# zacharie12/Hypernet-image-captioning

Hardware: AMD Instinct MI355X
Metric: training images/sec at 1/2/4/8 MI355X, Flickr30k GRU+hypernet bs=128 (higher is better)
Workload: dtype f32; 1 GPU; Flickr30k-shaped GRU+additive-attention decoder + hypernet (3 style domains), full training step (fwd, CE, bwd, clip 5.0, Adam); per_gpu_batch=128, global_batch=128, T=20, P=49, D=2048, F=200, E=200, H=200, V=9684, hypernet_params=144906720, parallelism=dp1, launch=eager, next_theta_in_adam_pass=True, next_precompute_beside_adam=True, spinup_steps=0, deterministic_gradients=True

## Files before the change

hypernet-image-captioning_amd/csrc/decoder.hip:

```cpp
#include "common.h"
#include "decoder_internal.h"
#include "gemm_internal.h"
#include <algorithm>
#include <initializer_list>
#include <mutex>

int g_tune_deterministic = 0;
int g_tune_rec_pair = 1;
int g_tune_rec_rotate = 1;
int g_tune_vocab_order = 1;
int g_tune_branch_mask = 7;
int g_tune_splitk_target = 1280;
int g_tune_chain_main = 0;
int g_tune_hops = 0;
int g_tune_fork = 4;
int g_tune_join_chain = 0;
int g_tune_sk_dhs = 0, g_tune_sk_vocab_w = 0;
#define RUN(x) do { int _rc = (x); if (_rc != CAPHN_OK) return _rc; } while (0)

namespace {

struct Side {
    hipStream_t st[3];
    enum { D_FORK = 0, D_JOIN = 1, D_X = 4, D_MS = 10, D_PRE_F = 14, D_PRE_ALL = 15, D_COUNT = 16 };
    struct Dep { hipEvent_t ev; unsigned seq = 0; bool by_value = false; };
    Dep deps[D_COUNT];
    unsigned* vals = nullptr;
    unsigned counter = 0;
    bool values = false;
    bool pre_valid = false;
    const void* pre_ws = nullptr;
    bool ready = false, on = false;
    bool forked[3] = {false, false, false};
    hipStream_t main = nullptr;
    int init() {
        if (ready) return CAPHN_OK;
        static std::mutex mu;
        std::lock_guard<std::mutex> lock(mu);
        if (ready) return CAPHN_OK;
        for (auto& s : st) if (hipStreamCreateWithFlags(&s, hipStreamNonBlocking) != hipSuccess) return CAPHN_ELAUNCH;
        for (auto& d : deps) if (hipEventCreateWithFlags(&d.ev, hipEventDisableTiming) != hipSuccess) return CAPHN_ELAUNCH;
        void* p = nullptr;
        if (hipMalloc(&p, sizeof(unsigned) * D_COUNT) == hipSuccess && hipMemset(p, 0, sizeof(unsigned) * D_COUNT) == hipSuccess)
            vals = static_cast<unsigned*>(p);
        else (void)hipGetLastError();
        ready = true;
        return CAPHN_OK;
    }
    int post(int slot, hipStream_t from) {
// ... 54 lines not shown
        return await(D_JOIN + i, st[j]);
    }
    struct Scope {
        Side& s;
        explicit Scope(Side& side) : s(side) {}
        ~Scope() { for (int i = 0; i < 3; ++i) if (s.on && s.forked[i]) (void)s.jointo(i); }
    };
    hipStream_t xfrom[6] = {nullptr, nullptr, nullptr, nullptr, nullptr, nullptr};
    int record(int k, hipStream_t from) {
        if (!on) return CAPHN_OK;
        xfrom[k] = from;
        return post(D_X + k, from);
    }
    int wait(int k, hipStream_t to) {
        if (!on || xfrom[k] == to) return CAPHN_OK;
        return await(D_X + k, to);
    }
    int dep(hipStream_t from, hipStream_t to, int k) {
        if (!on || from == to) return CAPHN_OK;
        if (post(D_X + k, from) != CAPHN_OK) return CAPHN_ELAUNCH;
        return await(D_X + k, to);
    }
};
constexpr int MAX_DEVICES = 64;
Side g_sides[MAX_DEVICES];
inline Side* side_here() {
    int dev = 0;
    if (hipGetDevice(&dev) != hipSuccess || dev < 0 || dev >= MAX_DEVICES) return nullptr;
    return &g_sides[dev];
}

struct Ws {
    size_t Y1, f, meanf, h0, c0, Waf, G, Xe, Xg, Hs, Hprev, gates, hn, Cs, Cprev, uah, alphas, idx;
    size_t dHs, dgi, dgh, duah, de, dh0, dc0, ctx, dctx, dXe, dWaf, dmeanf, df, dY1, apart, vtmp, colws, colws_s[3], prof, rowmap;
    size_t xch, xch_floats;
    size_t wp;
    size_t H0s, dH0, h0L, dcarry, tgi, tgh, tmpA, tmpB;
    size_t Lin[CAPHN_MAX_DEC_LAYERS - 1], Lgates[CAPHN_MAX_DEC_LAYERS - 1], Lhn[CAPHN_MAX_DEC_LAYERS - 1],
           Ldgi[CAPHN_MAX_DEC_LAYERS - 1], Ldgh[CAPHN_MAX_DEC_LAYERS - 1];
    int L1;
    size_t total;
    int npc, pchunk, NG, arows;
};
inline bool use_pair(const caphn_decoder_dims* d) {
    const int NG = d->cell == CAPHN_CELL_LSTM ? 4 : 3;
    return g_tune_rec_pair && d->T > 1 && d->layers <= 1 && caphn_rec_pair_resident_gates(d->P, d->H, NG) >= 0;
}

inline size_t up4(size_t v) { return (v + 3) & ~(size_t)3; }

inline Ws layout(const caphn_decoder_dims* d) {
    Ws w;
    const size_t B = d->B, T = d->T, P = d->P, F = d->F, E = d->E, H = d->H, V = d->V, D = d->D;
    const bool lstm = d->cell == CAPHN_CELL_LSTM, raw = d->raw_features != 0;
    const size_t NG = lstm ? 4 : 3;
    w.NG = (int)NG;
    size_t o = 0;
    auto take = [&](size_t n) { size_t r = o; o += up4(n); return r; };
    w.Y1 = take(raw ? 0 : B * P * F); w.f = take(raw ? 0 : B * P * F); w.meanf = take(B * F); w.h0 = take(B * H);
    w.c0 = take(lstm ? B * H : 0);
    w.Waf = take(B * P * H); w.G = take(B * P * NG * H); w.Xe = take(B * T * (E + F)); w.Xg = take(B * T * NG * H);
    w.Hs = take(B * T * H); w.Hprev = take(B * T * H); w.gates = take(B * T * NG * H); w.hn = take(lstm ? 0 : B * T * H);
    w.Cs = take(lstm ? B * T * H : 0); w.Cprev = take(lstm ? B * T * H : 0);
    w.uah = take(B * T * H); w.alphas = take(B * T * P); w.idx = take(2 * B * T);
    w.dHs = take(B * T * H); w.dgi = take(B * T * NG * H); w.dgh = take(lstm ? 0 : B * T * NG * H); w.duah = take(B * T * H);
    w.de = take(B * T * P); w.dh0 = take(B * H); w.dc0 = take(lstm ? B * H : 0);
    w.ctx = w.Xe + E; w.dctx = take(raw ? 0 : B * T * F);
    w.dXe = take(B * T * E); w.dWaf = take(B * P * H); w.dmeanf = take(raw ? 0 : 2 * B * F); w.df = take(raw ? 0 : B * P * F);
    w.dY1 = take(raw ? 0 : B * P * F);
    w.pchunk = 1; w.npc = (int)((P + w.pchunk - 1) / w.pchunk);
    const size_t arows = std::max<size_t>(std::max<size_t>(w.npc, (size_t)caphn_rec_bwd_groups((int)P, (int)H)),
                                          (size_t)caphn_rec_pair_bwd_groups((int)P, (int)H));
    w.arows = (int)arows;
    w.apart = take(B * arows * (H + 1)); w.vtmp = take(H + 1);
    size_t cs = 0;
    auto need = [&](size_t M, size_t N) { cs = std::max(cs, caphn_colsum_workspace_bytes((int)M, (int)N) / sizeof(float)); };
    need(B * T, V); need(B * T, NG * H); need(B * T, H); need(B * P, H); need(B * P, F); need(B, H);
    need(B * arows, H + 1);
    if (d->layers > 1) need(B * (T + 1), 3 * H);
    w.colws = take(cs);
    {
        size_t c2 = 0;
        auto need2 = [&](size_t M, size_t N) { c2 = std::max(c2, caphn_colsum_workspace_bytes((int)M, (int)N) / sizeof(float)); };
        need2(B * T, NG * H); need2(B * T, H); need2(B * P, H); need2(B * P, F); need2(B, H); need2(B * arows, H + 1);
        if (d->layers > 1) need2(B * (T + 1), 3 * H);
        for (int i = 0; i < 3; ++i) w.colws_s[i] = take(c2);
    }
    w.prof = take(64);
    w.rowmap = take(B * T + 4);
    w.xch_floats = caphn_rec_pair_xch_bytes((int)B, (int)P, (int)H) / sizeof(float);
    w.xch = take(2 * w.xch_floats);
    o = (o + 31) & ~(size_t)31;
    w.wp = take(caphn_rec_pair_wp_floats((int)H, (int)NG));
    w.L1 = d->layers > 1 ? d->layers - 1 : 0;
    {
        const size_t on = w.L1 > 0 ? 1 : 0, S = T + 1;
        w.H0s = take(on * B * T * H); w.dH0 = take(on * B * T * H); w.h0L = take(on * B * H); w.dcarry = take(on * B * H);
        w.tgi = take(on * B * 3 * H); w.tgh = take(on * B * 3 * H); w.tmpA = take(on * B * H); w.tmpB = take(on * B * H);
        for (int l = 0; l < CAPHN_MAX_DEC_LAYERS - 1; ++l) {
            const size_t u = l < w.L1 ? 1 : 0;
            w.Lin[l] = take(u * B * S * H); w.Lgates[l] = take(u * B * S * 3 * H); w.Lhn[l] = take(u * B * S * H);
            w.Ldgi[l] = take(u * B * S * 3 * H); w.Ldgh[l] = take(u * B * S * 3 * H);
        }
    }
    w.total = o;
    (void)D;
    return w;
}

__global__ __launch_bounds__(1024) void valid_rows_kernel(int n, const int64_t* __restrict__ tgt, int64_t ignore, int* __restrict__ map) {
    __shared__ int wsum[16];
    __shared__ int base_s;
    const int tid = threadIdx.x, lane = tid & 63, wave = tid >> 6;
    if (tid == 0) base_s = 0;
    __syncthreads();
    for (int c0 = 0; c0 < n; c0 += 1024) {
        const int i = c0 + tid;
        const int v = (i < n && tgt[i] != ignore) ? 1 : 0;
        const unsigned long long ball = __ballot(v);
        const int before = __popcll(ball & ((1ull << lane) - 1ull));
        if (lane == 0) wsum[wave] = __popcll(ball);
        __syncthreads();
        int woff = 0, tot = 0;
        for (int q = 0; q < 16; ++q) { if (q < wave) woff += wsum[q]; tot += wsum[q]; }
        const int base = base_s;
        if (v) map[4 + base + woff + before] = i;
        __syncthreads();
        if (tid == 0) base_s = base + tot;
        __syncthreads();
    }
    if (tid == 0) map[0] = base_s;
}

__global__ void copy2_kernel(const float* __restrict__ src, int n, float* __restrict__ a, float* __restrict__ b) {
    const int i = blockIdx.x * blockDim.x + threadIdx.x;
    if (i < n) a[i] = src[i];
    else if (i == n) b[0] = src[n];
}

__global__ __launch_bounds__(256) void teacher_inputs_kernel(int T, int E, const int64_t* __restrict__ caps, const float* __restrict__ table,
                                                            int64_t* __restrict__ idx, float* __restrict__ out, int ostride) {
    const int i = blockIdx.x, t = i % T;
    const int64_t id = t < 2 ? (int64_t)-1 : caps[i - 1];
    if (threadIdx.x == 0) idx[i] = id;
    for (int e = threadIdx.x; e < E; e += 256) out[(size_t)i * ostride + e] = id < 0 ? 0.f : table[(size_t)id * E + e];
}

inline bool dims_ok(const caphn_decoder_dims* d) {
    if (d && !(d->dropout_p >= 0.f && d->dropout_p < 1.f)) return false;
    if (!(d && d->B > 0 && d->T > 0 && d->P > 0 && d->D > 0 && d->F > 0 && d->E > 0 && d->H > 0 && d->V > 0)) return false;
    if (d->cell != CAPHN_CELL_GRU && d->cell != CAPHN_CELL_LSTM) return false;
    if (d->raw_features && d->F != d->D) return false;
    if (d->layers < 0 || d->layers > CAPHN_MAX_DEC_LAYERS) return false;
    if (d->layers > 1 && d->cell != CAPHN_CELL_GRU) return false;
    if (d->logits_ld != 0 && d->logits_ld < d->V) return false;
    return true;
}
inline bool layer_params_ok(const caphn_decoder_dims* d, const caphn_decoder_params* p) {
    for (int l = 0; l + 1 < d->layers; ++l)
        if (!p->lw_ih[l] || !p->lw_hh[l] || !p->lb_ih[l] || !p->lb_hh[l]) return false;
    return true;
}

inline int pick_splitk(int M, int N, int K) {
// ... 129 lines not shown
        a.dgi = ws + w.Ldgi[l]; a.dgh = ws + w.Ldgh[l]; a.dout = o; a.dout_ld = o_ld;
        if (l == w.L1 - 1 && slot > 0) { a.drop_p = d->dropout_p; a.drop_seed = d->dropout_seed; a.T = d->T; a.t = slot - 1; }
        RUN(caphn_launch_layer_gru_bwd(a, s));
        RUN(caphn_gemm_f32(0, 0, B, H, G3, ws + w.Ldgi[l] + (size_t)slot * G3, S * G3, p->lw_ih[l], H, o, o_ld, nullptr, nullptr, 0,
                           CAPHN_GEMM_ACCUM, 1, s));
        RUN(caphn_gemm_f32(0, 0, B, H, G3, ws + w.Ldgh[l] + (size_t)slot * G3, S * G3, p->lw_hh[l], H, o, o_ld, nullptr, nullptr, 0,
                           CAPHN_GEMM_ACCUM, 1, s));
        d1 = o; d1_ld = o_ld; d2 = nullptr;
    }
    return CAPHN_OK;
}

}

extern "C" size_t caphn_decoder_workspace_bytes(const caphn_decoder_dims* d) {
    if (!dims_ok(d)) return 0;
    return layout(d).total * sizeof(float);
}

extern "C" const int* caphn_decoder_rowcount_ptr(const caphn_decoder_dims* d, void* ws_) {
    if (!dims_ok(d) || !ws_) return nullptr;
    return reinterpret_cast<const int*>(static_cast<float*>(ws_) + layout(d).rowmap);
}

extern "C" unsigned long long* caphn_decoder_profile_ptr(const caphn_decoder_dims* d, void* ws_) {
    if (!dims_ok(d) || !ws_) return nullptr;
    return reinterpret_cast<unsigned long long*>(static_cast<float*>(ws_) + layout(d).prof);
}

extern "C" int caphn_decoder_prepare_rows(const caphn_decoder_dims* d, const int64_t* targets, int64_t ignore_index,
                                          void* ws_, caphn_stream_t stream) {
    if (!dims_ok(d) || !targets || !ws_) return CAPHN_EINVAL;
    const Ws w = layout(d);
    hipLaunchKernelGGL(valid_rows_kernel, dim3(1), dim3(1024), 0, static_cast<hipStream_t>(stream), d->B * d->T, targets,
                       ignore_index, reinterpret_cast<int*>(static_cast<float*>(ws_) + w.rowmap));
    return caphn_launch_status();
}

static int decoder_inputs(const caphn_decoder_dims* d, const caphn_decoder_params* p, const Ws& w, float* ws,
                          const int64_t* captions, hipStream_t s, int parts = 3) {
    const int BT = d->B * d->T, E = d->E, GH = w.NG * d->H, EF = d->E + d->F;
    int64_t* idx = reinterpret_cast<int64_t*>(ws + w.idx);
    if ((parts & 1) && !(d->precomputed & 64))
        hipLaunchKernelGGL(teacher_inputs_kernel, dim3(BT), dim3(256), 0, s, d->T, E, captions, p->embed_w, idx, ws + w.Xe, EF);
    if (parts & 2)
    RUN(caphn_gemm_f32(0, 1, BT, GH, E, ws + w.Xe, EF, p->w_ih, EF, ws + w.Xg, GH, p->b_ih, nullptr, 0, CAPHN_GEMM_BIAS, 1, s));
    return CAPHN_OK;
}

extern "C" int caphn_decoder_precompute(const caphn_decoder_dims* d, const caphn_decoder_params* p, const float* features,
                                        const int64_t* captions, void* ws_, caphn_stream_t stream) {
    if (!dims_ok(d) || !p || !features || !ws_) return CAPHN_EINVAL;
    const bool raw = d->raw_features != 0;
    if (!raw && (!p->fc0_w || !p->fc0_b || !p->fc2_w || !p->fc2_b)) return CAPHN_EINVAL;
    if (d->cell == CAPHN_CELL_LSTM && (!p->initc_w || !p->initc_b)) return CAPHN_EINVAL;
    const Ws w = layout(d);
    hipStream_t s = static_cast<hipStream_t>(stream);
    const float* f = nullptr;
    RUN(decoder_precompute(d, p, w, static_cast<float*>(ws_), features, &f, s, (captions ? 3 : 1) & ~(d->precomputed & 1), true));
    if (captions && !(d->precomputed & 4)) RUN(decoder_inputs(d, p, w, static_cast<float*>(ws_), captions, s));
    Side* sd = side_here();
    if (!sd || sd->post(Side::D_PRE_ALL, s) != CAPHN_OK) return CAPHN_ELAUNCH;
    sd->pre_valid = true;
    sd->pre_ws = ws_;
    return caphn_launch_status();
}

extern "C" int caphn_decoder_pair_prep(const caphn_decoder_dims* d, const caphn_decoder_params* p, void* ws_, caphn_stream_t stream) {
// ... 158 lines not shown

    const int* rmap = d->row_subset ? reinterpret_cast<const int*>(ws + w.rowmap) : nullptr;
    const int LV = d->logits_ld > 0 ? d->logits_ld : V;
    const int fork_mode = g_tune_fork == 4 ? (pair ? 2 : 1) : g_tune_fork;
    const bool late = fork_mode != 2;
    const bool gz = d->grads_zeroed != 0;
    const bool wg_first = !late && g_tune_vocab_order == 0;
    if (wg_first) {
        RUN(sd.forkto(0));
        RUN(wgrad_bias(V, H, BT, dlogits, LV, ws + w.Hs, H, g->out_w, H, g->out_b, rmap, cws, sd.s(0), gz));
        RUN(sd.milestone(CAPHN_MS_VOCAB, sd.s(0)));
    }
    const bool dhs_zero = (d->precomputed & 8) != 0;
    bool ctx_side = false;
    if (rmap) {
        if (!dhs_zero) RUN(caphn_zero_f32(ws + w.dHs, (size_t)BT * H, s));
        RUN(caphn_gemm_mapped(0, 0, BT, H, V, dlogits, LV, p->out_w, H, ws + w.dHs, H, nullptr, 0,
                              (g_tune_sk_dhs > 0 && !g_tune_deterministic) ? g_tune_sk_dhs : pick_splitk(BT, H, V),
                              rmap + 4, rmap, 1, s));
    } else
    RUN(gemm_auto(0, 0, BT, H, V, dlogits, LV, p->out_w, H, ws + w.dHs, H, nullptr, 0, s, nullptr, 0, dhs_zero));
    if (!late && !wg_first) {
        if (!(d->precomputed & 32) && sd.s(0) != s && sd.s(2) != s) {
            RUN(sd.fork_many({0, 2}));
            RUN(caphn_launch_ctx(B, T, P, F, ws + w.alphas, f, ws + w.ctx, EF, sd.s(2)));
            RUN(sd.record(5, sd.s(2)));
            ctx_side = true;
        } else
        RUN(sd.forkto(0));
        RUN(wgrad_bias(V, H, BT, dlogits, LV, ws + w.Hs, H, g->out_w, H, g->out_b, rmap, cws, sd.s(0), gz));
        RUN(sd.milestone(CAPHN_MS_VOCAB, sd.s(0)));
    }

    RecBwdArgs a;
    a.B = B; a.T = T; a.P = P; a.H = H; a.RG = RG;
    a.Waf = ws + w.Waf; a.G = ws + w.G; a.W_hh = p->w_hh; a.U_a = p->Ua_w; a.v_a = p->va_w;
    a.Hprev = ws + w.Hprev; a.alphas = ws + w.alphas; a.gates = ws + w.gates; a.hn = ws + w.hn; a.uah = ws + w.uah;
    a.Cs = ws + w.Cs; a.Cprev = ws + w.Cprev;
    a.dHs = ws + w.dHs; a.dalphas = dalphas;
    a.dgi = dgi; a.dgh = dgh; a.duah = ws + w.duah; a.de = ws + w.de; a.dh0 = ws + w.dh0; a.dc0 = ws + w.dc0;
    a.vecW = (H % 4 == 0) && caphn_aligned16(p->w_hh) && caphn_aligned16(p->Ua_w);
    a.vecS = (H % 4 == 0) && caphn_aligned16(ws);
    a.prof = reinterpret_cast<unsigned long long*>(ws + w.prof) + 8;
    a.rotate = g_tune_rec_rotate;
    a.drop_p = d->dropout_p; a.drop_seed = d->dropout_seed;
    const int ang = w.L1 > 0 ? 0 : pair ? caphn_rec_pair_bwd_groups(P, H) : caphn_rec_bwd_groups(P, H);
    if (ang > 0) { a.dWaf = ws + w.dWaf; a.apart = ws + w.apart; }
    if (w.L1 > 0) {
        RUN(caphn_zero_f32(ws + w.dcarry, (size_t)B * H, s));
        a.dHs = ws + w.dH0; a.dh0 = ws + w.dcarry; a.drop_p = 0.f;
        for (int t = T - 1; t >= 0; --t) {
            RUN(layers_backward(d, p, w, ws, t + 1, ws + w.dHs + (size_t)t * H, T * H, ws + w.dcarry, ws + w.dH0 + (size_t)t * H, T * H, s));
            a.t0 = t; a.t1 = t + 1;
            RUN(caphn_launch_rec_bwd(a, lstm, s));
        }
        RUN(layers_backward(d, p, w, ws, 0, ws + w.dcarry, H, nullptr, ws + w.dh0, H, s));
    } else if (pair) {
        a.xch = reinterpret_cast<unsigned long long*>(ws + w.xch) + w.xch_floats * sizeof(float) / sizeof(unsigned long long);
        a.apart_rows = ang;
        a.WP = ws + w.wp; a.wp_pitch = caphn_rec_pair_pitch(H);
        if (!raw) { a.inith_w = p->inith_w; a.initc_w = lstm ? p->initc_w : nullptr; a.dmean_part = ws + w.dmeanf; a.F = F; }
        RUN(caphn_launch_rec_pair_bwd(a, lstm, s));
    } else
    RUN(caphn_launch_rec_bwd(a, lstm, s));

    hipStream_t b0 = sd.s(0), b1 = sd.s(1), b2 = sd.s(2);
    const bool t_main = hook != nullptr && g_tune_chain_main != 0;
    hipStream_t sT = t_main ? s : b1, sF = t_main ? b1 : s;
    const bool hold_big = late && !raw && fork_mode == 3;
    RUN(sd.fork_many({0, 1, 2}));
    if (late && !hold_big) {
        RUN(wgrad_bias(V, H, BT, dlogits, LV, ws + w.Hs, H, g->out_w, H, g->out_b, rmap, cws, b0, gz));
        RUN(sd.milestone(CAPHN_MS_VOCAB, b0));
    }
    if (ctx_side) RUN(sd.wait(5, sT));
    else if (!(d->precomputed & 32)) RUN(caphn_launch_ctx(B, T, P, F, ws + w.alphas, f, ws + w.ctx, EF, sT));
    if (lstm) RUN(gemm_auto(1, 0, GH, EF, BT, dgi, GH, ws + w.Xe, EF, g->w_ih, EF, nullptr, 0, sT, nullptr, 0, gz));
    else RUN(wgrad_bias(GH, EF, BT, dgi, GH, ws + w.Xe, EF, g->w_ih, EF, g->b_ih, nullptr, cw1, sT, gz));
    RUN(wgrad_bias(GH, H, BT, dgh, GH, ws + w.Hprev, H, g->w_hh, H, g->b_hh, nullptr, cw2, b2, gz));
    if (lstm) RUN(caphn_colsum_f32(BT, GH, dgi, GH, g->b_ih, cw2, b2));
    RUN(sd.record(3, b2));
    hipStream_t se = late ? b2 : b0;
    RUN(caphn_gemm_f32(0, 0, BT, E, GH, dgi, GH, p->w_ih, EF, ws + w.dXe, E, nullptr, nullptr, 0, 0, 1, se));
    if (!gz) RUN(caphn_zero_f32(g->embed_w, (size_t)V * E, se));
    RUN(caphn_embedding_scatter_add_v(BT, E, V, ws + w.dXe, idx, g->embed_w, se));
    RUN(sd.milestone(CAPHN_MS_EMBED, se));
    RUN(sd.wait(3, sT));
    RUN(sd.milestone(CAPHN_MS_DTHETA, sT));
    if (hook && !hold_big) {
        RUN(caphn_hyper_backward(hook->hd, g->w_ih, hook->acts, hook->hg, hook->ws, sT));
    }
    if (!hold_big) RUN(sd.milestone(CAPHN_MS_HYPER, sT));
    if (!raw) {
        RUN(caphn_gemm_f32(0, 0, BT, F, GH, dgi, GH, p->w_ih + E, EF, ws + w.dctx, F, nullptr, nullptr, 0, 0, 1, sF));
        if (!pair)
            RUN(caphn_launch_dmean(B, H, F, ws + w.dh0, p->inith_w, lstm ? ws + w.dc0 : nullptr, lstm ? p->initc_w : nullptr,
                                   ws + w.dmeanf, sF));
    }
    AttnGradArgs ag;
    ag.T = T; ag.P = P; ag.H = H; ag.pchunk = w.pchunk;
    ag.Waf = ws + w.Waf; ag.uah = ws + w.uah; ag.de = ws + w.de; ag.v_a = p->va_w;
    ag.dWaf = ws + w.dWaf; ag.part = ws + w.apart;
    if (ang == 0) RUN(caphn_launch_attn_param_grads(ag, B, w.npc, sF));
    RUN(sd.record(2, sF));
    RUN(wgrad_bias(H, H, BT, ws + w.duah, H, ws + w.Hprev, H, g->Ua_w, H, g->Ua_b, nullptr, cws, b0, gz));
    for (int l = 0; l < w.L1; ++l) {
        const int BS = B * (T + 1), G3 = 3 * H;
        RUN(wgrad_bias(G3, H, BS, ws + w.Ldgi[l], G3, ws + w.Lin[l], H, g->lw_ih[l], H, g->lb_ih[l], nullptr, cws, b0, gz));
        RUN(wgrad_bias(G3, H, BS, ws + w.Ldgh[l], G3, ws + w.Lin[l], H, g->lw_hh[l], H, g->lb_hh[l], nullptr, cws, b0, gz));
    }
    RUN(wgrad_bias(H, F, B, ws + w.dh0, H, ws + w.meanf, F, g->inith_w, F, g->inith_b, nullptr, cws, b0, gz));
    if (lstm) RUN(wgrad_bias(H, F, B, ws + w.dc0, H, ws + w.meanf, F, g->initc_w, F, g->initc_b, nullptr, cws, b0, gz));
    if (!raw) {
        RUN(caphn_launch_df(B, T, P, F, ws + w.alphas, ws + w.dctx, ws + w.dmeanf, ws + w.df, sF, pair ? ws + w.dmeanf + (size_t)B * F : nullptr));
        RUN(caphn_gemm_f32(0, 0, BP, F, H, ws + w.dWaf, H, p->Wa_w, F, ws + w.df, F, nullptr, nullptr, 0, CAPHN_GEMM_ACCUM, 1, sF));
        RUN(sd.record(4, sF));
        if (hold_big) {
            RUN(sd.wait(4, b0));
            RUN(wgrad_bias(V, H, BT, dlogits, LV, ws + w.Hs, H, g->out_w, H, g->out_b, rmap, cws, b0, gz));
            RUN(sd.milestone(CAPHN_MS_VOCAB, b0));
            if (hook) {
                RUN(sd.wait(4, sT));
                RUN(caphn_hyper_backward(hook->hd, g->w_ih, hook->acts, hook->hg, hook->ws, sT));
            }
            RUN(sd.milestone(CAPHN_MS_HYPER, sT));
        }
        RUN(caphn_gemm_f32(0, 0, BP, F, F, ws + w.df, F, p->fc2_w, F, ws + w.dY1, F, nullptr, ws + w.Y1, F, CAPHN_GEMM_MASK, 1, sF));
        RUN(wgrad_bias(F, D, BP, ws + w.dY1, F, features, D, g->fc0_w, D, g->fc0_b, nullptr, cw0, sF, gz));
    }
    RUN(sd.wait(2, b2));
    RUN(caphn_colsum_f32(B * (ang > 0 ? ang : w.npc), H + 1, ws + w.apart, H + 1, ws + w.vtmp, cw2, b2));
    hipLaunchKernelGGL(copy2_kernel, dim3((H + 256) / 256), dim3(256), 0, b2, ws + w.vtmp, H, g->va_w, g->va_b);
    RUN(wgrad_bias(H, F, BP, ws + w.dWaf, H, f, F, g->Wa_w, F, g->Wa_b, nullptr, cw2, b2, gz));
    if (!raw) {
        RUN(sd.wait(4, b2));
        RUN(wgrad_bias(F, F, BP, ws + w.df, F, ws + w.Y1, F, g->fc2_w, F, g->fc2_b, nullptr, cw2, b2, gz));
    }
    if (g_tune_join_chain) { RUN(sd.join_into(0, 1)); RUN(sd.join_into(2, 1)); RUN(sd.jointo(1)); }
// ... 244 lines not shown
```

hypernet-image-captioning_amd/csrc/decoder_internal.h:

```cpp
#pragma once
#include "common.h"

struct RecFwdArgs {
    int B, T, P, H;
    int RG;
    const float* Waf;
    const float* G;
    const float* Xg;
    const float* h0;
    const float* c0;
    const float* W_hh; const float* b_hh;
    const float* U_a; const float* b_Ua;
    const float* v_a; const float* b_va;
    float* Hs; float* Hprev;
    float* alphas;
    float* gates;
    float* hn;
    float* Cs; float* Cprev;
    float* uah;
    unsigned long long* prof;
    int vecW, vecS, rotate;
    int slab_div = 1;
    unsigned long long* xch = nullptr;
    const float* WP = nullptr; int wp_pitch = 0;
    int t0 = 0, t1 = 0;
    float drop_p = 0.f; unsigned long long drop_seed = 0;
    int waf_lds = 0;
    int wc_rows = 0;
    unsigned epoch = 0; int* err = nullptr; long long xlimit = 0;
    const float* Hsrc = nullptr;
};
struct RecBwdArgs {
    int B, T, P, H;
    int RG;
    const float* Waf; const float* G;
    const float* W_hh; const float* U_a; const float* v_a;
    const float* Hprev; const float* alphas; const float* gates; const float* hn; const float* uah;
    const float* Cs; const float* Cprev;
    const float* dHs;
    const float* dalphas;
    float* dgi; float* dgh;
    float* duah;
    float* de;
    float* dh0;
    float* dc0;
    unsigned long long* prof;
    int vecW, vecS, rotate;
    float* dWaf = nullptr; float* apart = nullptr;
    unsigned long long* xch = nullptr;
    const float* WP = nullptr; int wp_pitch = 0;
    int apart_rows = 0;
    float drop_p = 0.f; unsigned long long drop_seed = 0;
    unsigned epoch = 0; int* err = nullptr; long long xlimit = 0;
    const float* inith_w = nullptr; const float* initc_w = nullptr; float* dmean_part = nullptr; int F = 0;
    int part_rows = 0, wc_rows = 0;
    int t0 = 0, t1 = 0;
};
struct AttnGradArgs {
    int T, P, H, pchunk;
    const float* Waf; const float* uah; const float* de; const float* v_a;
    float* dWaf;
    float* part;
};

struct LayerFwdArgs {
    int B, H, S, slot;
    const float* gi; const float* gh;
    const float* hin; int hin_ld;
    float* hout; int hout_ld;
    float* sin; float* sgates; float* shn;
    float drop_p = 0.f; unsigned long long drop_seed = 0; int T = 1, t = 0;
};
struct LayerBwdArgs {
    int B, H, S, slot;
    const float* d1; int d1_ld; const float* d2;
    const float* sin; const float* sgates; const float* shn;
    float* dgi; float* dgh;
    float* dout; int dout_ld;
    float drop_p = 0.f; unsigned long long drop_seed = 0; int T = 1, t = 0;
};
int caphn_launch_layer_gru_fwd(const LayerFwdArgs& a, hipStream_t s);
int caphn_launch_layer_gru_bwd(const LayerBwdArgs& a, hipStream_t s);

size_t caphn_rec_fwd_lds_bytes(int P, int H, int NG, int RG);
size_t caphn_rec_bwd_lds_bytes(int P, int H, int NG, int RG);
int caphn_rec_resident_gates(int P, int H, int NG);
int caphn_launch_rec_fwd(const RecFwdArgs& a, bool lstm, hipStream_t s);
int caphn_launch_rec_bwd(const RecBwdArgs& a, bool lstm, hipStream_t s);
bool caphn_rec_pair_ok(int P, int H, int NG, int RG);
// ... 40 lines not shown
```

hypernet-image-captioning_amd/csrc/hyper.hip:

```cpp
#include "common.h"
#include <algorithm>

namespace {

constexpr float LRELU = 0.01f;
__device__ __forceinline__ float lrelu(float v) { return v > 0.f ? v : LRELU * v; }
__device__ __forceinline__ float lrelu_grad(float post) { return post > 0.f ? 1.f : LRELU; }

struct GemvJob {
    const float* W; const float* b; const float* x; float* y;
    int rows, k, act, vec;
    int block0, nblocks;
    float* xcopy;
};
struct GemvJobs { GemvJob j[CAPHN_MAX_HEADS]; int n; };

template <int QMAX, int RB, bool NTL>
__device__ __forceinline__ void gemv_rows_wave(const GemvJob& J, int wave_g, int nwaves, int lane) {
    const int k4 = J.k >> 2;
    const f32x4* x4 = reinterpret_cast<const f32x4*>(J.x);
    f32x4 xr[QMAX];
#pragma unroll
    for (int q = 0; q < QMAX; ++q) {
        int c = lane + 64 * q;
// ... 795 lines not shown

extern "C" int caphn_outer_f32(int rows, int k, const float* gv, const float* av, float* out, caphn_stream_t stream) {
    if (rows <= 0 || k <= 0 || !gv || !av || !out) return CAPHN_EINVAL;
    OuterJobs o2; o2.n = 1;
    OuterJob& J = o2.j[0];
    J.g = gv; J.a = av; J.out = out; J.rows = rows; J.k = k; J.block0 = 0;
    long nb = ((long)rows * k + 1023) / 1024;
    hipLaunchKernelGGL(outer_kernel, dim3((unsigned)nb), dim3(256), 0, static_cast<hipStream_t>(stream), o2);
    return caphn_launch_status();
}

extern int g_tune_adam;
extern int g_tune_gemm;
extern int g_tune_rec_rotate;
extern int g_tune_fork;
extern int g_tune_gemm_xcd;
extern int g_tune_gemm_fast;
extern int g_tune_gemm_planes;
extern int g_tune_rec_pair;
extern int g_tune_gemm_single;
extern int g_tune_gemm_tile;
extern int g_tune_deterministic;
extern int g_tune_adam_cap;
extern int g_tune_chain_main;
extern int g_tune_rec_cache;
extern int g_tune_splitk_target;
extern int g_tune_gemm_order;
extern int g_tune_branch_mask;
extern int g_tune_gemm_db;
extern int g_tune_gemm_ws;
extern int g_tune_adam_dense_cap;
extern int g_tune_sk_dhs, g_tune_sk_vocab_w;
extern int g_tune_join_chain;
extern int g_tune_gemm_kres;
extern int g_tune_gemm_waves;
extern int g_tune_hops;
extern int g_tune_vocab_order;
extern int g_det_vocab;
int caphn_rec_pair_debug_skip(int v);
int caphn_rec_pair_debug_opts(int v);
extern "C" int caphn_tune(int key, int value) {
    if (key == 0) { g_tune_gemv = value; return CAPHN_OK; }
    if (key == 1) { g_tune_adam = value; return CAPHN_OK; }
    if (key == 2) { g_tune_gemm = value; return CAPHN_OK; }
    if (key == 3) { g_tune_rec_rotate = value; return CAPHN_OK; }
    if (key == 4) { g_tune_fork = value; return CAPHN_OK; }
    if (key == 6) { g_tune_gemm_xcd = value; return CAPHN_OK; }
    if (key == 7) { g_tune_gemm_fast = value; return CAPHN_OK; }
    if (key == 8) { g_tune_gemm_planes = value; return CAPHN_OK; }
    if (key == 9) { g_tune_rec_pair = value; return CAPHN_OK; }
    if (key == 10) return caphn_rec_pair_debug_skip(value);
    if (key == 11) { g_tune_gemm_single = value; return CAPHN_OK; }
    if (key == 12) { g_tune_gemm_tile = value; return CAPHN_OK; }
    if (key == 13) { g_tune_deterministic = value > 0; g_det_vocab = value; return CAPHN_OK; }
    if (key == 21) { g_tune_vocab_order = value != 0; return CAPHN_OK; }
    if (key == 20) { if (value < 0 || value > 7) return CAPHN_EINVAL; g_tune_branch_mask = value; return CAPHN_OK; }
    if (key == 18) { if (value < 0 || value > 2) return CAPHN_EINVAL; g_tune_gemm_order = value; return CAPHN_OK; }
    if (key == 17) { if (value < 1 || value > 65536) return CAPHN_EINVAL; g_tune_splitk_target = value; return CAPHN_OK; }
    if (key == 16) { if (value < 0 || value > 2) return CAPHN_EINVAL; g_tune_rec_cache = value; return CAPHN_OK; }
    if (key == 15) { g_tune_chain_main = value != 0; return CAPHN_OK; }
    if (key == 26) { g_tune_hops = value != 0; return CAPHN_OK; }
    if (key == 27) { g_tune_hyper_tail = value != 0; return CAPHN_OK; }
    if (key == 28) { g_tune_acts_fused = value != 0; return CAPHN_OK; }
    if (key == 36) { g_tune_gemm_kres = value != 0; return CAPHN_OK; }
    if (key == 35) { g_tune_join_chain = value != 0; return CAPHN_OK; }
    if (key == 33) { if (value < 0 || value > 64) return CAPHN_EINVAL; g_tune_sk_dhs = value; return CAPHN_OK; }
    if (key == 34) { if (value < 0 || value > 64) return CAPHN_EINVAL; g_tune_sk_vocab_w = value; return CAPHN_OK; }
    if (key == 30) { if (value < 64 || value > 4096) return CAPHN_EINVAL; g_tune_vjp_blocks = value; return CAPHN_OK; }
    if (key == 31) { if (value < 64 || value > 65535) return CAPHN_EINVAL; g_tune_adam_dense_cap = value; return CAPHN_OK; }
    if (key == 29) { if (value != 0 && value != 64 && value != 128) return CAPHN_EINVAL; g_tune_gemm_ws = value; return CAPHN_OK; }
    if (key == 25) { if (value != 0 && value != 5 && value != 6) return CAPHN_EINVAL; g_tune_gemm_waves = value; return CAPHN_OK; }
    if (key == 24) return caphn_rec_pair_debug_opts(value);
    if (key == 23) { if (value < 0 || value > 7) return CAPHN_EINVAL; g_tune_gemm_db = value; return CAPHN_OK; }
    if (key == 22) { if (value < 1) return CAPHN_EINVAL; g_tune_xch_timeout = 100ll * value; return CAPHN_OK; }
    if (key == 14) { if (value < 64 || value > 65535) return CAPHN_EINVAL; g_tune_adam_cap = value; return CAPHN_OK; }
    return CAPHN_EINVAL;
}
```

hypernet-image-captioning_amd/csrc/recurrent_pair.hip:

```cpp
#include "common.h"
#include "decoder_internal.h"
#include <atomic>

namespace {

constexpr int NT = 512;
#ifdef CAPHN_REC_PROFILE
#define PSTAMP(i) do { if (prof_on) { unsigned long long _n = clock64(); pc[i] += _n - plast; plast = _n; } } while (0)
#define PDECL const bool prof_on = (w == 0 && tid == 0 && a.prof != nullptr); \
    unsigned long long pc[8] = {0, 0, 0, 0, 0, 0, 0, 0}, plast = prof_on ? clock64() : 0
#define PFLUSH do { if (prof_on) for (int i = 0; i < 8; ++i) a.prof[i] = pc[i]; } while (0)
#else
#define PSTAMP(i) do { } while (0)
#define PDECL do { } while (0)
#define PFLUSH do { } while (0)
#endif

typedef unsigned long long u64;

__device__ int d_pair_opts = 0;
__device__ __forceinline__ void xsend(u64* slot, float v, unsigned tag, bool near = false) {
    const u64 bits = ((u64)tag << 32) | (u64)__float_as_uint(v);
    if (near) __hip_atomic_store(slot, bits, __ATOMIC_RELAXED, __HIP_MEMORY_SCOPE_WORKGROUP);
    else __hip_atomic_store(slot, bits, __ATOMIC_RELAXED, __HIP_MEMORY_SCOPE_AGENT);
// ... 469 lines not shown
    float* duah_s = va_s + nkm;
    float* dgh_s = duah_s + nk;
    float* dgi_s = duah_s + (NG + 1) * nkm;
    float* dal_s = dgi_s + NG * nkm;
    float* al_s = dal_s + Ppad;
    float* dhp_s = al_s + Ppad;
    float* part_s = dhp_s + H4;
    float* Wc_s = part_s + (size_t)a.part_rows * H4;

    u64* xmine = a.xch + (size_t)w * xch_stride(P, H);
    u64* xpart = a.xch + (size_t)(w ^ 8) * xch_stride(P, H);
    u64* xh_mine = xmine; u64* xe_mine = xmine + nkm;
    u64* xh_part = xpart; u64* xe_part = xpart + nkm;
    const unsigned ep = a.epoch << 16;
    const XCtl xc{a.err, a.xlimit};
    const bool mute = d_skip_xrecv == 2 && hh == 1;
    const bool near = partner_is_near(xmine + xch_ctl(P, H), xpart + xch_ctl(P, H), ep | 0xFFFFu, a.err, a.xlimit, tid, reinterpret_cast<int*>(dal_s));

    const float* Gb = a.G + (size_t)b * P * GH;
    const int vecS = a.vecS && (nk % 4 == 0) && (k0 % 4 == 0);
    if (vecS) {
        const int n4 = nk >> 2;
        for (int i = tid; i < P * RG * n4; i += NT) {
            const int c = i % n4, pq = i / n4, q = pq % RG, p = pq / RG;
            reinterpret_cast<f32x4*>(G_s + (size_t)pq * nk)[c] = reinterpret_cast<const f32x4*>(Gb + (size_t)p * GH + q * H + k0)[c];
        }
    } else {
        for (int i = tid; i < P * RG * nk; i += NT) {
            const int kk = i % nk, pq = i / nk, q = pq % RG, p = pq / RG;
            G_s[(size_t)pq * nk + kk] = Gb[(size_t)p * GH + q * H + k0 + kk];
        }
    }
    const int bt0 = a.t0, bt1 = a.t1 > 0 ? a.t1 : T;
    for (int kk = tid; kk < nk; kk += NT) {
        dh_s[kk] = 0.f; va_s[kk] = a.v_a[k0 + kk];
        dc_s[kk] = (LSTM && bt1 < T) ? a.dc0[(size_t)b * H + k0 + kk] : 0.f;
    }
    const float* Waf_b = a.Waf + (size_t)b * P * H;
    const int CH = (H % 4) == 0 ? 4 : 1;
    const KG m = kg_map(tid, nk);
    const int NR = (NG + 1) * nk;
    __syncthreads();
    const bool fuse = a.dWaf != nullptr && m.g >= 0;
    float dw[PGM];
#pragma unroll
    for (int i = 0; i < PGM; ++i) dw[i] = 0.f;
    float wafr[PGM];
#pragma unroll
    for (int i = 0; i < PGM; ++i) { const int p = m.g + i * m.ng; wafr[i] = (fuse && p < P) ? Waf_b[p * H + k0 + m.k] : 0.f; }
    float dva = 0.f, dbva = 0.f;
    PDECL;

    f32x4 wreg[TCR > 0 ? TCR : 1];
    const int tc_nch = (H + 3) / 4, tc_nsl = NT / (tc_nch < NT ? tc_nch : NT);
    const int tc_chunk = tid % tc_nch, tc_slice = tid / tc_nch;
    if constexpr (TCR > 0) {
#pragma unroll
        for (int u = 0; u < TCR; ++u) {
            const int r = a.wc_rows + tc_slice + u * tc_nsl;
            wreg[u] = (tc_slice < tc_nsl && r < NR) ? *reinterpret_cast<const f32x4*>(WPh + (size_t)r * a.wp_pitch + tc_chunk * 4)
                                                     : f32x4{0.f, 0.f, 0.f, 0.f};
        }
    }
    const float* dvec_s = duah_s;
    auto tmatvec = [&](int cb, int ce) {
        if constexpr (TCR > 0) {
// ... 76 lines not shown
                if (CH == 4) *reinterpret_cast<f32x4*>(part_s + (size_t)slice * H4 + c * 4) = f32x4{acc[0], acc[1], acc[2], acc[3]};
                else part_s[(size_t)slice * H4 + c] = acc[0];
            }
        }
        __syncthreads();
        for (int j = tid; j < ncol; j += NT) {
            float sum = 0.f;
            for (int sl = 0; sl < nsl; ++sl) sum += part_s[(size_t)sl * H4 + j];
            dhp_s[cb + j] = sum;
        }
        __syncthreads();
    };
    if (a.wc_rows > 0) {
        const int n4 = H >> 2;
        for (int idx = tid; idx < a.wc_rows * n4; idx += NT) {
            const int r = idx / n4, c = idx - r * n4;
            reinterpret_cast<f32x4*>(Wc_s)[idx] = reinterpret_cast<const f32x4*>(WPh + (size_t)r * a.wp_pitch)[c];
        }
        __syncthreads();
    }
    const bool pfk = nk <= NT && P <= NT;
    float pf[8] = {0.f, 0.f, 0.f, 0.f, 0.f, 0.f, 0.f, 0.f}, pfa = 0.f;
    auto prefetch = [&](int t) {
        const size_t bt = (size_t)b * T + t;
        if (tid < P) pfa = a.alphas[bt * P + tid];
        if (tid < nk) {
            const int k = k0 + tid;
            pf[0] = a.dHs[bt * H + k]; pf[1] = a.uah[bt * H + k];
            pf[2] = a.gates[bt * GH + k]; pf[3] = a.gates[bt * GH + H + k]; pf[4] = a.gates[bt * GH + 2 * H + k];
            if (LSTM) { pf[5] = a.gates[bt * GH + (3 % NG) * H + k]; pf[6] = a.Cprev[bt * H + k]; pf[7] = a.Cs[bt * H + k]; }
            else { pf[5] = a.hn[bt * H + k]; pf[6] = a.Hprev[bt * H + k]; }
        }
    };
    if (pfk) prefetch(bt1 - 1);

    for (int t = bt1 - 1; t >= bt0; --t) {
        const size_t bt = (size_t)b * T + t;
        if (pfk) { if (tid < P) al_s[tid] = pfa; }
        else for (int p = tid; p < P; p += NT) al_s[p] = a.alphas[bt * P + p];
        for (int kk = tid; kk < nk; kk += NT) {
            const int k = k0 + kk;
            float dh = dh_s[kk] + (pfk ? pf[0] : a.dHs[bt * H + k]);
            if (a.drop_p > 0.f) dh *= caphn_keep_scale(a.drop_seed, (unsigned long long)bt * H + k, a.drop_p, 1.0f / (1.0f - a.drop_p));
            uah_s[kk] = pfk ? pf[1] : a.uah[bt * H + k];
            if (LSTM) {
                const float gi = pfk ? pf[2] : a.gates[bt * GH + k], gf = pfk ? pf[3] : a.gates[bt * GH + H + k];
                const float gg = pfk ? pf[4] : a.gates[bt * GH + 2 * H + k];
                const float go = pfk ? pf[5] : a.gates[bt * GH + (3 % NG) * H + k];
                const float cp = pfk ? pf[6] : a.Cprev[bt * H + k];
                const float tc = caphn_tanh(pfk ? pf[7] : a.Cs[bt * H + k]);
                const float d_o = dh * tc;
                const float dc = dc_s[kk] + dh * go * (1.0f - tc * tc);
                const float dip = dc * gg * gi * (1.0f - gi);
                const float dfp = dc * cp * gf * (1.0f - gf);
                const float dgp = dc * gi * (1.0f - gg * gg);
                const float dop = d_o * go * (1.0f - go);
                dc_s[kk] = dc * gf;
                dh_s[kk] = 0.f;
                dgi_s[kk] = dip; dgi_s[nk + kk] = dfp; dgi_s[2 * nk + kk] = dgp; dgi_s[(3 % NG) * nk + kk] = dop;
                dgh_s[kk] = dip; dgh_s[nk + kk] = dfp; dgh_s[2 * nk + kk] = dgp; dgh_s[(3 % NG) * nk + kk] = dop;
                a.dgi[bt * GH + k] = dip; a.dgi[bt * GH + H + k] = dfp; a.dgi[bt * GH + 2 * H + k] = dgp;
                a.dgi[bt * GH + (3 % NG) * H + k] = dop;
            } else {
                const float r = pfk ? pf[2] : a.gates[bt * GH + k], z = pfk ? pf[3] : a.gates[bt * GH + H + k];
                const float n = pfk ? pf[4] : a.gates[bt * GH + 2 * H + k];
                const float hnv = pfk ? pf[5] : a.hn[bt * H + k], hp = pfk ? pf[6] : a.Hprev[bt * H + k];
                const float dn = dh * (1.0f - z);
                const float dz = dh * (hp - n);
                const float dnp = dn * (1.0f - n * n);
// ... 375 lines not shown
```

Before: 49990 images/s.

## Skip padded trailing timesteps in recurrent BPTT and optionally in weight-grad GEMMs

Computes a per-sequence live length, the last non-ignored target, plus a compacted map of live (b,t) steps in the row-prep kernel. The paired recurrent backward kernel starts its reverse loop at each sequence's live length and zero-fills the gate, attention and energy gradients for the padded tail. This removes serial BPTT steps that only carry zero gradient. An optional, off-by-default flag also restricts the weight/bias gradient GEMMs to live rows. The prep kernel gains an extra compaction pass.

```diff
diff --git a/hypernet-image-captioning_amd/csrc/decoder.hip b/hypernet-image-captioning_amd/csrc/decoder.hip
--- a/hypernet-image-captioning_amd/csrc/decoder.hip
+++ b/hypernet-image-captioning_amd/csrc/decoder.hip
@@ -15,6 +15,8 @@
 int g_tune_hops = 0;
 int g_tune_fork = 4;
 int g_tune_join_chain = 0;
+int g_tune_bptt_live = 1;
+int g_tune_wgrad_live = 0;
 int g_tune_sk_dhs = 0, g_tune_sk_vocab_w = 0;
 #define RUN(x) do { int _rc = (x); if (_rc != CAPHN_OK) return _rc; } while (0)
 
@@ -135,7 +137,7 @@
 
 struct Ws {
     size_t Y1, f, meanf, h0, c0, Waf, G, Xe, Xg, Hs, Hprev, gates, hn, Cs, Cprev, uah, alphas, idx;
-    size_t dHs, dgi, dgh, duah, de, dh0, dc0, ctx, dctx, dXe, dWaf, dmeanf, df, dY1, apart, vtmp, colws, colws_s[3], prof, rowmap;
+    size_t dHs, dgi, dgh, duah, de, dh0, dc0, ctx, dctx, dXe, dWaf, dmeanf, df, dY1, apart, vtmp, colws, colws_s[3], prof, rowmap, live, stepmap;
     size_t xch, xch_floats;
     size_t wp;
     size_t H0s, dH0, h0L, dcarry, tgi, tgh, tmpA, tmpB;
@@ -191,6 +193,8 @@
     }
     w.prof = take(64);
     w.rowmap = take(B * T + 4);
+    w.live = take(B);
+    w.stepmap = take(B * T + 4);
     w.xch_floats = caphn_rec_pair_xch_bytes((int)B, (int)P, (int)H) / sizeof(float);
     w.xch = take(2 * w.xch_floats);
     o = (o + 31) & ~(size_t)31;
@@ -211,28 +215,39 @@
     return w;
 }
 
-__global__ __launch_bounds__(1024) void valid_rows_kernel(int n, const int64_t* __restrict__ tgt, int64_t ignore, int* __restrict__ map) {
+__global__ __launch_bounds__(1024) void valid_rows_kernel(int n, int T, const int64_t* __restrict__ tgt, int64_t ignore, int* __restrict__ map,
+                                                          int* __restrict__ live, int* __restrict__ smap) {
     __shared__ int wsum[16];
     __shared__ int base_s;
     const int tid = threadIdx.x, lane = tid & 63, wave = tid >> 6;
-    if (tid == 0) base_s = 0;
-    __syncthreads();
-    for (int c0 = 0; c0 < n; c0 += 1024) {
-        const int i = c0 + tid;
-        const int v = (i < n && tgt[i] != ignore) ? 1 : 0;
-        const unsigned long long ball = __ballot(v);
-        const int before = __popcll(ball & ((1ull << lane) - 1ull));
-        if (lane == 0) wsum[wave] = __popcll(ball);
+    for (int b = tid; b < n / T; b += 1024) {
+        int t = T;
+        while (t > 0 && tgt[(size_t)b * T + t - 1] == ignore) --t;
+        live[b] = t;
+    }
+    auto compact = [&](auto keep, int* __restrict__ out) {
+        if (tid == 0) base_s = 0;
         __syncthreads();
-        int woff = 0, tot = 0;
-        for (int q = 0; q < 16; ++q) { if (q < wave) woff += wsum[q]; tot += wsum[q]; }
-        const int base = base_s;
-        if (v) map[4 + base + woff + before] = i;
+        for (int c0 = 0; c0 < n; c0 += 1024) {
+            const int i = c0 + tid;
+            const int v = (i < n && keep(i)) ? 1 : 0;
+            const unsigned long long ball = __ballot(v);
+            const int before = __popcll(ball & ((1ull << lane) - 1ull));
+            if (lane == 0) wsum[wave] = __popcll(ball);
+            __syncthreads();
+            int woff = 0, tot = 0;
+            for (int q = 0; q < 16; ++q) { if (q < wave) woff += wsum[q]; tot += wsum[q]; }
+            const int base = base_s;
+            if (v) out[4 + base + woff + before] = i;
+            __syncthreads();
+            if (tid == 0) base_s = base + tot;
+            __syncthreads();
+        }
+        if (tid == 0) out[0] = base_s;
         __syncthreads();
-        if (tid == 0) base_s = base + tot;
-        __syncthreads();
-    }
-    if (tid == 0) map[0] = base_s;
+    };
+    compact([&](int i) { return tgt[i] != ignore; }, map);
+    compact([&](int i) { return i % T < live[i / T]; }, smap);
 }
 
 __global__ void copy2_kernel(const float* __restrict__ src, int n, float* __restrict__ a, float* __restrict__ b) {
@@ -428,8 +443,10 @@
                                           void* ws_, caphn_stream_t stream) {
     if (!dims_ok(d) || !targets || !ws_) return CAPHN_EINVAL;
     const Ws w = layout(d);
-    hipLaunchKernelGGL(valid_rows_kernel, dim3(1), dim3(1024), 0, static_cast<hipStream_t>(stream), d->B * d->T, targets,
-                       ignore_index, reinterpret_cast<int*>(static_cast<float*>(ws_) + w.rowmap));
+    float* ws = static_cast<float*>(ws_);
+    hipLaunchKernelGGL(valid_rows_kernel, dim3(1), dim3(1024), 0, static_cast<hipStream_t>(stream), d->B * d->T, d->T, targets,
+                       ignore_index, reinterpret_cast<int*>(ws + w.rowmap), reinterpret_cast<int*>(ws + w.live),
+                       reinterpret_cast<int*>(ws + w.stepmap));
     return caphn_launch_status();
 }
 
@@ -654,6 +671,8 @@
         RUN(sd.milestone(CAPHN_MS_VOCAB, sd.s(0)));
     }
 
+    const bool live_ok = d->row_subset && dalphas == nullptr && pair && w.L1 == 0;
+    const int* smap = (live_ok && g_tune_wgrad_live) ? reinterpret_cast<const int*>(ws + w.stepmap) : nullptr;
     RecBwdArgs a;
     a.B = B; a.T = T; a.P = P; a.H = H; a.RG = RG;
     a.Waf = ws + w.Waf; a.G = ws + w.G; a.W_hh = p->w_hh; a.U_a = p->Ua_w; a.v_a = p->va_w;
@@ -678,6 +697,7 @@
         }
         RUN(layers_backward(d, p, w, ws, 0, ws + w.dcarry, H, nullptr, ws + w.dh0, H, s));
     } else if (pair) {
+        if (live_ok && g_tune_bptt_live) a.live = reinterpret_cast<const int*>(ws + w.live);
         a.xch = reinterpret_cast<unsigned long long*>(ws + w.xch) + w.xch_floats * sizeof(float) / sizeof(unsigned long long);
         a.apart_rows = ang;
         a.WP = ws + w.wp; a.wp_pitch = caphn_rec_pair_pitch(H);
@@ -698,8 +718,8 @@
     if (ctx_side) RUN(sd.wait(5, sT));
     else if (!(d->precomputed & 32)) RUN(caphn_launch_ctx(B, T, P, F, ws + w.alphas, f, ws + w.ctx, EF, sT));
     if (lstm) RUN(gemm_auto(1, 0, GH, EF, BT, dgi, GH, ws + w.Xe, EF, g->w_ih, EF, nullptr, 0, sT, nullptr, 0, gz));
-    else RUN(wgrad_bias(GH, EF, BT, dgi, GH, ws + w.Xe, EF, g->w_ih, EF, g->b_ih, nullptr, cw1, sT, gz));
-    RUN(wgrad_bias(GH, H, BT, dgh, GH, ws + w.Hprev, H, g->w_hh, H, g->b_hh, nullptr, cw2, b2, gz));
+    else RUN(wgrad_bias(GH, EF, BT, dgi, GH, ws + w.Xe, EF, g->w_ih, EF, g->b_ih, smap, cw1, sT, gz));
+    RUN(wgrad_bias(GH, H, BT, dgh, GH, ws + w.Hprev, H, g->w_hh, H, g->b_hh, smap, cw2, b2, gz));
     if (lstm) RUN(caphn_colsum_f32(BT, GH, dgi, GH, g->b_ih, cw2, b2));
     RUN(sd.record(3, b2));
     hipStream_t se = late ? b2 : b0;
@@ -725,7 +745,7 @@
     ag.dWaf = ws + w.dWaf; ag.part = ws + w.apart;
     if (ang == 0) RUN(caphn_launch_attn_param_grads(ag, B, w.npc, sF));
     RUN(sd.record(2, sF));
-    RUN(wgrad_bias(H, H, BT, ws + w.duah, H, ws + w.Hprev, H, g->Ua_w, H, g->Ua_b, nullptr, cws, b0, gz));
+    RUN(wgrad_bias(H, H, BT, ws + w.duah, H, ws + w.Hprev, H, g->Ua_w, H, g->Ua_b, smap, cws, b0, gz));
     for (int l = 0; l < w.L1; ++l) {
         const int BS = B * (T + 1), G3 = 3 * H;
         RUN(wgrad_bias(G3, H, BS, ws + w.Ldgi[l], G3, ws + w.Lin[l], H, g->lw_ih[l], H, g->lb_ih[l], nullptr, cws, b0, gz));
diff --git a/hypernet-image-captioning_amd/csrc/decoder_internal.h b/hypernet-image-captioning_amd/csrc/decoder_internal.h
--- a/hypernet-image-captioning_amd/csrc/decoder_internal.h
+++ b/hypernet-image-captioning_amd/csrc/decoder_internal.h
@@ -55,6 +55,7 @@
     const float* inith_w = nullptr; const float* initc_w = nullptr; float* dmean_part = nullptr; int F = 0;
     int part_rows = 0, wc_rows = 0;
     int t0 = 0, t1 = 0;
+    const int* live = nullptr;
 };
 struct AttnGradArgs {
     int T, P, H, pchunk;
diff --git a/hypernet-image-captioning_amd/csrc/hyper.hip b/hypernet-image-captioning_amd/csrc/hyper.hip
--- a/hypernet-image-captioning_amd/csrc/hyper.hip
+++ b/hypernet-image-captioning_amd/csrc/hyper.hip
@@ -851,6 +851,7 @@
 extern int g_tune_adam_dense_cap;
 extern int g_tune_sk_dhs, g_tune_sk_vocab_w;
 extern int g_tune_join_chain;
+extern int g_tune_bptt_live, g_tune_wgrad_live;
 extern int g_tune_gemm_kres;
 extern int g_tune_gemm_waves;
 extern int g_tune_hops;
@@ -883,6 +884,8 @@
     if (key == 28) { g_tune_acts_fused = value != 0; return CAPHN_OK; }
     if (key == 36) { g_tune_gemm_kres = value != 0; return CAPHN_OK; }
     if (key == 35) { g_tune_join_chain = value != 0; return CAPHN_OK; }
+    if (key == 37) { g_tune_bptt_live = value != 0; return CAPHN_OK; }
+    if (key == 38) { g_tune_wgrad_live = value != 0; return CAPHN_OK; }
     if (key == 33) { if (value < 0 || value > 64) return CAPHN_EINVAL; g_tune_sk_dhs = value; return CAPHN_OK; }
     if (key == 34) { if (value < 0 || value > 64) return CAPHN_EINVAL; g_tune_sk_vocab_w = value; return CAPHN_OK; }
     if (key == 30) { if (value < 64 || value > 4096) return CAPHN_EINVAL; g_tune_vjp_blocks = value; return CAPHN_OK; }
diff --git a/hypernet-image-captioning_amd/csrc/recurrent_pair.hip b/hypernet-image-captioning_amd/csrc/recurrent_pair.hip
--- a/hypernet-image-captioning_amd/csrc/recurrent_pair.hip
+++ b/hypernet-image-captioning_amd/csrc/recurrent_pair.hip
@@ -525,6 +525,35 @@
         }
     }
     const int bt0 = a.t0, bt1 = a.t1 > 0 ? a.t1 : T;
+    const int btl = a.live ? max(bt0, min(bt1, a.live[b])) : bt1;
+    if (btl < bt1) {
+        const int nt = bt1 - btl;
+        float* dgi_b = a.dgi + ((size_t)b * T + btl) * GH;
+        float* dgh_b = a.dgh + ((size_t)b * T + btl) * GH;
+        float* duah_b = a.duah + ((size_t)b * T + btl) * H;
+        if (vecS) {
+            const int n4 = nk >> 2;
+            const f32x4 z4 = {0.f, 0.f, 0.f, 0.f};
+            for (int i = tid; i < nt * (NG + 1) * n4; i += NT) {
+                const int c = i % n4, tq = i / n4, q = tq % (NG + 1), tt = tq / (NG + 1);
+                if (q == NG) reinterpret_cast<f32x4*>(duah_b + (size_t)tt * H + k0)[c] = z4;
+                else {
+                    reinterpret_cast<f32x4*>(dgi_b + (size_t)tt * GH + q * H + k0)[c] = z4;
+                    if (!LSTM) reinterpret_cast<f32x4*>(dgh_b + (size_t)tt * GH + q * H + k0)[c] = z4;
+                }
+            }
+        } else {
+            for (int i = tid; i < nt * (NG + 1) * nk; i += NT) {
+                const int kk = i % nk, tq = i / nk, q = tq % (NG + 1), tt = tq / (NG + 1);
+                if (q == NG) duah_b[(size_t)tt * H + k0 + kk] = 0.f;
+                else {
+                    dgi_b[(size_t)tt * GH + q * H + k0 + kk] = 0.f;
+                    if (!LSTM) dgh_b[(size_t)tt * GH + q * H + k0 + kk] = 0.f;
+                }
+            }
+        }
+        if (hh == 0) for (int i = tid; i < nt * P; i += NT) a.de[((size_t)b * T + btl) * P + i] = 0.f;
+    }
     for (int kk = tid; kk < nk; kk += NT) {
         dh_s[kk] = 0.f; va_s[kk] = a.v_a[k0 + kk];
         dc_s[kk] = (LSTM && bt1 < T) ? a.dc0[(size_t)b * H + k0 + kk] : 0.f;
@@ -667,9 +696,9 @@
             else { pf[5] = a.hn[bt * H + k]; pf[6] = a.Hprev[bt * H + k]; }
         }
     };
-    if (pfk) prefetch(bt1 - 1);
-
-    for (int t = bt1 - 1; t >= bt0; --t) {
+    if (pfk && btl > bt0) prefetch(btl - 1);
+
+    for (int t = btl - 1; t >= bt0; --t) {
         const size_t bt = (size_t)b * T + t;
         if (pfk) { if (tid < P) al_s[tid] = pfa; }
         else for (int p = tid; p < P; p += NT) al_s[p] = a.alphas[bt * P + p];
```

Result: no change. 49780 images/s (-0.4%).
